# succinctlabs/sp1

Hardware: AMD Instinct MI355X
Metric: RISC-V cycles proved/sec (core shard prove): whole ShardProof of a full core shard of the reference's `fibonacci` guest, see config (higher is better)
Workload: dtype u32 (KoalaBear Montgomery words, exact integer arithmetic)

## Files before the change

sp1_amd/csrc/zc_compile.hpp:

```cpp
#pragma once
#include <memory>
#include <vector>

#include "common.hpp"
#include "zc_device.hpp"
#include "zc_poseidon2.hpp"
#include "zc_keccak.hpp"
#include "zc_mul.hpp"
#include "zc_poly.hpp"

namespace sp1hip {

using Ext = kb::Ext;
static inline Ext operator+(const Ext& a, const Ext& b) { return kb::ext_add(a, b); }
static inline Ext operator-(const Ext& a, const Ext& b) { return kb::ext_sub(a, b); }
static inline Ext operator*(const Ext& a, const Ext& b) { return kb::ext_mul(a, b); }

struct ZcMacro {
    uint32_t kind, base_col, first_constraint, aux0 = 0, aux1 = 0;
    uint32_t n_c = 0;
    uint32_t n_constraints() const { return kind == ZC_HINT_POLY ? n_c : kind == ZC_HINT_POSEIDON2 ? ZC_P2_CONSTRAINTS : kind == ZC_HINT_KECCAK ? ZC_KK_CONSTRAINTS : kind == ZC_HINT_MUL ? ZC_MUL_CONSTRAINTS : kind == ZC_HINT_SEPTIC_CURVE ? 7u : 14u; }
    uint32_t n_pieces() const { return kind == ZC_HINT_POLY ? 1u : kind == ZC_HINT_POSEIDON2 ? ZC_P2_PIECES : kind == ZC_HINT_KECCAK ? ZC_KK_PIECES : kind == ZC_HINT_MUL ? ZC_MUL_PIECES : kind == ZC_HINT_SEPTIC_CURVE ? 2u : 4u; }
    uint32_t n_host_pieces() const { return kind == ZC_HINT_SEPTIC_CURVE ? 1u : kind == ZC_HINT_SEPTIC_SUM ? 2u : n_pieces(); }
    void owned(uint32_t* lo, uint32_t* n) const {
        if (kind == ZC_HINT_POLY) { *lo = 0; *n = 0; }
        else if (kind == ZC_HINT_POSEIDON2) { *lo = base_col; *n = ZC_P2_COLUMNS; }
        else if (kind == ZC_HINT_KECCAK) { *lo = base_col; *n = ZC_KK_COLUMNS; }
        else if (kind == ZC_HINT_MUL) { *lo = base_col + MUL_CARRY; *n = ZC_MUL_OWNED; }
        else if (kind == ZC_HINT_SEPTIC_CURVE) { *lo = base_col; *n = 14; }
        else { *lo = aux0; *n = 28; }
    }
};

struct Chunk {
    std::vector<uint32_t> prog;
    uint32_t n_regs = 1, alpha_off = 0;
};

struct ZcPlan {
    uint32_t n_instr = 0, main_w = 0, prep_w = 0;
    bool macros_enabled = true;
    bool mul_enabled = true;
    std::vector<uint32_t> source;
    std::vector<uint32_t> prog;
    uint32_t n_regs = 1;
    std::vector<Chunk> chunks, mono, fine;
    std::vector<uint32_t> sched;
    std::vector<ZcMacro> macros;
    std::vector<ZcPoly> polys;
    std::vector<std::vector<ZcPolySeg>> poly_segs;
};

constexpr uint32_t ZC_FINE_LIMIT = 32, ZC_FINE_MAX_TERMS = 64;

int zc_get_plan(const uint32_t* program, uint32_t n_instr, uint32_t main_width, uint32_t prep_width, int chip_index,
                std::shared_ptr<const ZcPlan>* out, uint64_t rows = ~0ull);

Ext zc_eval_zero_row(const ZcPlan& plan, const Ext* alpha_pows, const uint32_t* publics);

}
```

sp1_amd/csrc/zc_kernels.hpp:

```cpp
#pragma once
#include "device_ctx.hpp"
#include "round_sync.hpp"
#include "zc_device.hpp"
#include "zc_poseidon2.hpp"
#include "zc_keccak.hpp"
#include "zc_mul.hpp"
#include "zc_poly.hpp"

namespace sp1hip {

template <bool FIRST, int MAXR> struct RegFile;

typedef uint32_t zc_lds_word_t __attribute__((address_space(3)));
typedef uint32_t zc_lds_quad_t __attribute__((ext_vector_type(4), address_space(3)));
typedef uint32_t zc_quad_t __attribute__((ext_vector_type(4)));
template <> struct RegFile<true, 0> {
    zc_lds_word_t* base;
    uint32_t stride;
    __device__ __forceinline__ uint32_t get(uint32_t i) const { return base[i * stride]; }
    __device__ __forceinline__ void set(uint32_t i, uint32_t v) { base[i * stride] = v; }
};
template <> struct RegFile<false, 0> {
    zc_lds_quad_t* base;
    uint32_t stride;
// ... 437 lines not shown
            const uint32_t k = threadIdx.x;
            partial[((size_t)bid * ZC_BIV_NODES + 4 * grp + n) * 8 + k] = kb::add(kb::add(red[k], red[8 + k]), kb::add(red[16 + k], red[24 + k]));
        }
    }
}

constexpr uint32_t ZC_CORNER_COLS = 32;
__global__ __launch_bounds__(256) void zc_biv_corner_kernel(const ZcDesc* __restrict__ descs, int n_descs, const uint32_t* __restrict__ eq,
                                                            uint32_t eq_len, uint32_t* __restrict__ partial, uint32_t block_base) {
    using K = KT<true>;
    __shared__ uint32_t red[4 * 16];
    const uint32_t bid = block_base + blockIdx.x;
    const ZcDesc d = zc_find_desc(descs, n_descs, bid);
    const uint32_t c0 = d.aux0, c1 = d.aux1;
    const uint32_t quads = (d.rows + 3) / 4;
    kb::Ext sb[4] = {kb::ext_zero(), kb::ext_zero(), kb::ext_zero(), kb::ext_zero()};
    for (uint32_t base = (bid - d.block_start) * d.block_pairs; base < quads; base += d.n_blocks * d.block_pairs)
    for (uint32_t i = base + threadIdx.x; i < min(base + d.block_pairs, quads); i += blockDim.x) {
        kb::Ext e;
#pragma unroll
        for (int k = 0; k < 4; k++) e.c[k] = eq[(size_t)k * eq_len + i];
        kb::Ext vb[4] = {kb::ext_zero(), kb::ext_zero(), kb::ext_zero(), kb::ext_zero()};
#pragma unroll 4
        for (uint32_t c = c0; c < c1; c++) {
            const kb::Ext pw = load_ext_aos(d.gkr_pows, c);
            const uint32_t* tbl = c < d.main_w ? d.main : d.prep;
            const uint32_t col = c < d.main_w ? c : c - d.main_w;
#pragma unroll
            for (uint32_t n = 0; n < 4; n++)
                if (4 * i + n < d.rows) vb[n] = kb::ext_add(vb[n], K::scale(pw, K::load(tbl, col, d.rows, 4 * i + n)));
        }
#pragma unroll
        for (int n = 0; n < 4; n++) sb[n] = kb::ext_add(sb[n], kb::ext_mul(vb[n], e));
    }
    const int lane = threadIdx.x & 63, wave = threadIdx.x >> 6;
#pragma unroll
    for (int n = 0; n < 4; n++)
#pragma unroll
        for (int k = 0; k < 4; k++) {
            const uint32_t w = zc_wave_sum(sb[n].c[k]);
            if (lane == 0) red[wave * 16 + 4 * n + k] = w;
        }
    __syncthreads();
    if (threadIdx.x < ZC_BIV_NODES * 8) {
        const uint32_t node = threadIdx.x / 8, k = threadIdx.x % 8;
        uint32_t v = 0;
        if (node < 4 && k >= 4) {
            const uint32_t j = 4 * node + (k - 4);
            v = kb::add(kb::add(red[j], red[16 + j]), kb::add(red[32 + j], red[48 + j]));
        }
        partial[((size_t)bid * ZC_BIV_NODES + node) * 8 + k] = v;
    }
}

template <uint32_t KIND>
__global__ __launch_bounds__(256) void zc_biv_macro_kernel(const ZcDesc* __restrict__ descs, int n_descs, const uint32_t* __restrict__ eq,
                                                           uint32_t eq_len, uint32_t* __restrict__ partial, uint32_t block_base,
                                                           const p2::RoundConstants* __restrict__ rc_p) {
    using K = KT<true>;
    __shared__ uint32_t red[32];
    if (threadIdx.x < 32) red[threadIdx.x] = 0;
    const uint32_t bid = block_base + blockIdx.x / (uint32_t)ZC_BIV_NODES;
    const uint32_t node = blockIdx.x % (uint32_t)ZC_BIV_NODES;
    const ZcBivNode nd = zc_biv_node(node);
    const ZcDesc d = zc_find_desc(descs, n_descs, bid);
    const uint32_t q = (d.flags >> 8) & 15u, base_col = d.pad;
    const auto* rc = (const p2::RoundConstants __attribute__((address_space(4)))*)(uintptr_t)rc_p;
    __syncthreads();
    const uint32_t quads = (d.rows + 3) / 4;
    kb::Ext sa = kb::ext_zero();
    for (uint32_t base = (bid - d.block_start) * d.block_pairs; base < quads; base += d.n_blocks * d.block_pairs)
    for (uint32_t i = base + threadIdx.x; i < min(base + d.block_pairs, quads); i += blockDim.x) {
        kb::Ext e;
#pragma unroll
        for (int k = 0; k < 4; k++) e.c[k] = eq[(size_t)k * eq_len + i];
        kb::Ext va = kb::ext_zero();
        auto ld_at = [&](uint32_t col, bool) -> uint32_t { return zc_biv_leaf(d.main, col, d.rows, i, nd); };
        auto ld = [&](uint32_t c, bool owned) -> uint32_t { return ld_at(base_col + c, owned); };
        auto sink = [&](uint32_t j, const uint32_t& v) { va = kb::ext_add(va, K::scale(load_ext_aos(d.alpha_pows, d.alpha_off + j), v)); };
        auto alpha = [&](uint32_t j) -> kb::Ext { return load_ext_aos(d.alpha_pows, d.alpha_off + j); };
        auto emit = [&](const kb::Ext& v) { va = kb::ext_add(va, v); };
        if constexpr (KIND == ZC_HINT_POSEIDON2) zc_p2_piece<P2Base>(q, rc, ld, sink);
        else if constexpr (KIND == ZC_HINT_KECCAK) zc_keccak_piece<P2Base>(q, ld, sink);
        else if constexpr (KIND == ZC_HINT_MUL) zc_mul_piece<P2Base>(q, ld, [&](uint32_t c, bool owned) -> uint32_t { return ld_at(d.aux0 + c, owned); }, sink);
        else if constexpr (KIND == ZC_HINT_SEPTIC_CURVE) zc_septic_curve_piece_w<P2Base, K>(q, ld, alpha, emit);
        else zc_septic_sum_piece_w<P2Base, K>(q, ld, [&](uint32_t c, bool owned) -> uint32_t { return ld_at(d.aux0 + c, owned); },
                                              [&]() -> uint32_t { return ld_at(d.aux1, false); }, alpha, emit);
        sa = kb::ext_add(sa, kb::ext_mul(va, e));
    }
    const int lane = threadIdx.x & 63, wave = threadIdx.x >> 6;
    uint32_t v[4];
#pragma unroll
    for (int k = 0; k < 4; k++) v[k] = zc_wave_sum(sa.c[k]);
    __syncthreads();
    if (lane == 0) {
#pragma unroll
        for (int k = 0; k < 4; k++) red[wave * 8 + k] = v[k];
    }
    __syncthreads();
    if (threadIdx.x < 8) {
        const uint32_t k = threadIdx.x;
        partial[((size_t)bid * ZC_BIV_NODES + node) * 8 + k] = k < 4 ? kb::add(kb::add(red[k], red[8 + k]), kb::add(red[16 + k], red[24 + k])) : 0u;
    }
}

struct ZcPolyTable {
    zc_const_words_t tb;
    __device__ __forceinline__ uint32_t word(uint32_t off) const { return tb[off]; }
    __device__ __forceinline__ kb::Ext coef(uint32_t off) const { return kb::Ext{{tb[off + 4], tb[off + 5], tb[off + 6], tb[off + 7]}}; }
};
__device__ __forceinline__ kb::Ext zc_ext_times_pow2(kb::Ext v, uint32_t k) {
    if (k == 0) return kb::ext_zero();
    for (uint32_t m = 1; m < k; m <<= 1) v = kb::ext_add(v, v);
    return v;
}
template <bool FIRST>
__global__ __launch_bounds__(256) void zc_poly_kernel(const ZcDesc* __restrict__ descs, int n_descs, const uint32_t* __restrict__ eq,
                                                      uint32_t eq_len, uint32_t* __restrict__ partial, uint32_t block_base) {
    using K = KT<FIRST>;
    using T = typename K::T;
    __shared__ uint32_t red[4 * 24];
    const uint32_t bid = block_base + blockIdx.x;
    const ZcDesc d = zc_find_desc(descs, n_descs, bid);
    const ZcPolyTable tab{(zc_const_words_t)(uintptr_t)d.prog};
    const uint32_t n_terms = tab.word(0), n_rest = tab.word(1), n_owned = tab.word(2);
    const uint32_t terms = (d.rows + 1) / 2;
    kb::Ext sa[3] = {kb::ext_zero(), kb::ext_zero(), kb::ext_zero()}, sb[2] = {kb::ext_zero(), kb::ext_zero()};
    for (uint32_t base = (bid - d.block_start) * d.block_pairs; base < terms; base += d.n_blocks * d.block_pairs)
    for (uint32_t i = base + threadIdx.x; i < min(base + d.block_pairs, terms); i += blockDim.x) {
        kb::Ext e;
#pragma unroll
        for (int k = 0; k < 4; k++) e.c[k] = eq[(size_t)k * eq_len + i];
        const bool has1 = 2 * i + 1 < d.rows;
        uint32_t off = ZC_POLY_HDR;
        auto form = [&](uint32_t n, kb::Ext& f0, kb::Ext& f1) {
            f0 = f1 = tab.coef(off);
            off += ZC_POLY_ENTRY;
#pragma unroll 4
            for (uint32_t k = 0; k < n; k++, off += ZC_POLY_ENTRY) {
                const uint32_t col = tab.word(off);
                const kb::Ext c = tab.coef(off);
                const T x0 = K::load(d.main, col, d.rows, 2 * i);
                const T x1 = has1 ? K::load(d.main, col, d.rows, 2 * i + 1) : K::zero();
                f0 = kb::ext_add(f0, K::scale(c, x0));
                f1 = kb::ext_add(f1, K::scale(c, x1));
            }
        };
        kb::Ext v0 = kb::ext_zero(), v2 = kb::ext_zero(), v4 = kb::ext_zero();
        for (uint32_t t = 0; t < n_terms; t++) {
            kb::Ext a0, a1, b0, b1;
            form(tab.word(4 + 3 * t), a0, a1);
            form(tab.word(5 + 3 * t), b0, b1);
            a0 = kb::ext_mul(a0, e); a1 = kb::ext_mul(a1, e);
            const kb::Ext da = kb::ext_sub(a1, a0), db = kb::ext_sub(b1, b0);
            const kb::Ext da2 = kb::ext_add(da, da), db2 = kb::ext_add(db, db);
            const kb::Ext a2 = kb::ext_add(a0, da2), b2 = kb::ext_add(b0, db2);
            kb::Ext p0 = FIRST ? kb::ext_zero() : kb::ext_mul(a0, b0), p2 = kb::ext_mul(a2, b2), p4 = kb::ext_mul(kb::ext_add(a2, da2), kb::ext_add(b2, db2));
            const uint32_t n2 = tab.word(6 + 3 * t);
            if (n2 != ZC_POLY_NONE) {
                kb::Ext c0, c1;
                form(n2, c0, c1);
                const kb::Ext dc = kb::ext_sub(c1, c0), dc2 = kb::ext_add(dc, dc), c2 = kb::ext_add(c0, dc2);
                if (!FIRST) p0 = kb::ext_mul(p0, c0);
                p2 = kb::ext_mul(p2, c2);
                p4 = kb::ext_mul(p4, kb::ext_add(c2, dc2));
            }
            v0 = kb::ext_add(v0, p0); v2 = kb::ext_add(v2, p2); v4 = kb::ext_add(v4, p4);
// ... 209 lines not shown
        for (int k = 0; k < 4; k++) rr[k] = kb::ext_mul(rr[k], e);
        slopes(rr);
#pragma unroll
        for (int n = 0; n < ZC_BIV_NODES; n++) sa[n] = kb::ext_add(sa[n], at(rr, zc_biv_node(n)));
    }
    const int lane = threadIdx.x & 63, wave = threadIdx.x >> 6;
    uint32_t v[48];
#pragma unroll
    for (int n = 0; n < ZC_BIV_NODES; n++)
#pragma unroll
        for (int k = 0; k < 4; k++) v[n * 4 + k] = zc_wave_sum(sa[n].c[k]);
    if (lane == 0) {
#pragma unroll
        for (int k = 0; k < 48; k++) red[wave * 48 + k] = v[k];
    }
    __syncthreads();
    if (threadIdx.x < 48) {
        const uint32_t k = threadIdx.x;
        uint32_t acc = red[k];
        for (uint32_t w = 1; w < blockDim.x / 64; w++) acc = kb::add(acc, red[w * 48 + k]);
        partial[((size_t)bid * ZC_BIV_NODES + k / 4) * 8 + (k & 3u)] = acc;
        partial[((size_t)bid * ZC_BIV_NODES + k / 4) * 8 + 4 + (k & 3u)] = 0u;
    }
}

struct P2Base4 {
    using T = kb::Ext;
    static __device__ __forceinline__ T add(const T& a, const T& b) { return kb::ext_add(a, b); }
    static __device__ __forceinline__ T sub(const T& a, const T& b) { return kb::ext_sub(a, b); }
    static __device__ __forceinline__ T mul(const T& a, const T& b) { return KT4::mul(a, b); }
    static __device__ __forceinline__ T addc(const T& a, uint32_t c) { return KC4::addc(a, c); }
    static __device__ __forceinline__ T mulc(const T& a, uint32_t c) { return kb::ext_mul_base(a, c); }
};
__global__ __launch_bounds__(256) void zc_biv_keccak_kernel(const ZcDesc* __restrict__ descs, int n_descs, const uint32_t* __restrict__ eq,
                                                            uint32_t eq_len, uint32_t* __restrict__ partial, uint32_t block_base) {
    using K = KT<true>;
    __shared__ uint32_t red[4][32];
    const uint32_t bid = block_base + blockIdx.x / ZC_BIV_GROUPS;
    const uint32_t grp = blockIdx.x % ZC_BIV_GROUPS;
    const ZcBivNode n0 = zc_biv_node(4 * grp), n1 = zc_biv_node(4 * grp + 1), n2 = zc_biv_node(4 * grp + 2), n3 = zc_biv_node(4 * grp + 3);
    const ZcDesc d = zc_find_desc(descs, n_descs, bid);
    const uint32_t q = (d.flags >> 8) & 15u, base_col = d.pad;
    const uint32_t quads = (d.rows + 3) / 4;
    kb::Ext sa[4] = {kb::ext_zero(), kb::ext_zero(), kb::ext_zero(), kb::ext_zero()};
    for (uint32_t base = (bid - d.block_start) * d.block_pairs; base < quads; base += d.n_blocks * d.block_pairs)
    for (uint32_t i = base + threadIdx.x; i < min(base + d.block_pairs, quads); i += blockDim.x) {
        kb::Ext e;
#pragma unroll
        for (int k = 0; k < 4; k++) e.c[k] = eq[(size_t)k * eq_len + i];
        kb::Ext va[4] = {kb::ext_zero(), kb::ext_zero(), kb::ext_zero(), kb::ext_zero()};
        auto ld = [&](uint32_t c, bool) -> kb::Ext {
            const zc_global_words_t g = (zc_global_words_t)d.main + (size_t)(base_col + c) * d.rows;
            const uint32_t r = 4 * i;
            const uint32_t r00 = g[r], r01 = r + 1 < d.rows ? g[r + 1] : 0u, r10 = r + 2 < d.rows ? g[r + 2] : 0u, r11 = r + 3 < d.rows ? g[r + 3] : 0u;
            return kb::Ext{{zc_biv_interp(r00, r01, r10, r11, n0), zc_biv_interp(r00, r01, r10, r11, n1), zc_biv_interp(r00, r01, r10, r11, n2),
                            zc_biv_interp(r00, r01, r10, r11, n3)}};
        };
        auto sink = [&](uint32_t j, const kb::Ext& v) {
            const kb::Ext a = load_ext_aos(d.alpha_pows, d.alpha_off + j);
#pragma unroll
            for (int n = 0; n < 4; n++) va[n] = kb::ext_add(va[n], K::scale(a, v.c[n]));
        };
        zc_keccak_piece<P2Base4>(q, ld, sink);
#pragma unroll
        for (int n = 0; n < 4; n++) sa[n] = kb::ext_add(sa[n], kb::ext_mul(va[n], e));
    }
    const int lane = threadIdx.x & 63, wave = threadIdx.x >> 6;
#pragma unroll
    for (int n = 0; n < 4; n++)
#pragma unroll
        for (int k = 0; k < 4; k++) {
            const uint32_t v = zc_wave_sum(sa[n].c[k]);
            if (lane == 0) red[wave][n * 4 + k] = v;
        }
    __syncthreads();
    if (threadIdx.x < 32) {
        const uint32_t n = threadIdx.x >> 3, k = threadIdx.x & 7u;
        const uint32_t w = n * 4 + (k & 3u);
        partial[((size_t)bid * ZC_BIV_NODES + 4 * grp + n) * 8 + k] =
            k < 4 ? kb::add(kb::add(red[0][w], red[1][w]), kb::add(red[2][w], red[3][w])) : 0u;
    }
}

constexpr uint32_t ZC_BIV_SUM_WORDS = 68;
__global__ __launch_bounds__(256) void zc_biv_reduce_kernel(const ZcChipRange* __restrict__ ranges, const uint32_t* __restrict__ partial,
                                                            const uint32_t* __restrict__ eq, uint32_t eq_len,
                                                            uint32_t* __restrict__ out, RoundSync rs, uint32_t seq) {
    __shared__ uint32_t acc[32][8];
    const uint32_t range = blockIdx.x / (uint32_t)ZC_BIV_NODES, node = blockIdx.x % (uint32_t)ZC_BIV_NODES;
    const ZcChipRange d = ranges[range];
    const uint32_t word = threadIdx.x & 7u, grp = threadIdx.x >> 3;
    {
        const uint32_t* p = partial + ((size_t)d.block_start * ZC_BIV_NODES + node) * 8 + word;
        uint32_t a[4] = {0, 0, 0, 0};
        uint32_t b = grp;
        for (; b + 96 < d.n_blocks; b += 128)
#pragma unroll
            for (int u = 0; u < 4; u++) a[u] = kb::add(a[u], p[(size_t)(b + 32 * u) * (ZC_BIV_NODES * 8)]);
        for (; b < d.n_blocks; b += 32) a[0] = kb::add(a[0], p[(size_t)b * (ZC_BIV_NODES * 8)]);
        acc[grp][word] = kb::add(kb::add(a[0], a[1]), kb::add(a[2], a[3]));
    }
    __syncthreads();
    if (threadIdx.x < 12) {
        const uint32_t w = threadIdx.x;
        uint32_t val = 0, dst = 0xffffffffu;
        if (w < 8) {
            for (uint32_t g = 0; g < 32; g++) val = kb::add(val, acc[g][w]);
            if (w < 4) dst = 4 * node + w;
            else if (node < 4) dst = 48 + 4 * node + (w - 4);
        } else if (node == 0) {
            const uint32_t k = w - 8;
            val = d.th < eq_len ? eq[(size_t)k * eq_len + d.th] : 0u;
            dst = 64 + k;
        }
        if (dst != 0xffffffffu) {
            out[(size_t)range * ZC_BIV_SUM_WORDS + dst] = val;
            if (rs.host_slot != nullptr)
                __hip_atomic_store(const_cast<uint32_t*>(rs.host_slot) + 1 + (size_t)range * ZC_BIV_SUM_WORDS + dst, val, __ATOMIC_RELAXED, __HIP_MEMORY_SCOPE_SYSTEM);
        }
    }
    if (rs.host_slot == nullptr) return;
    asm volatile("s_waitcnt vmcnt(0)" ::: "memory");
    __syncthreads();
    if (threadIdx.x == 0 && rs_ticket_is_last_acq_rel(rs.counter, blockIdx.x, gridDim.x)) rs_publish_seq(rs.host_slot, seq);
}

template <bool FIRST>
__global__ __launch_bounds__(256) void zc_reduce_kernel(const ZcChipRange* __restrict__ ranges, const uint32_t* __restrict__ partial,
                                                        const uint32_t* __restrict__ eq, uint32_t eq_len,
                                                        uint32_t* __restrict__ out, RoundSync rs, uint32_t seq) {
    __shared__ uint32_t acc[10][24];
    const ZcChipRange d = ranges[blockIdx.x];
    uint32_t y0, y2, y4, e;
    zc_reduce_range<FIRST>(d, partial, eq, eq_len, acc, y0, y2, y4, e);
    if (threadIdx.x < 4) {
        const uint32_t k = threadIdx.x;
        uint32_t* o = out + (size_t)blockIdx.x * 16;
        o[k] = y0; o[4 + k] = y2; o[8 + k] = y4;
        o[12 + k] = e;
    }
    if (rs.host_slot != nullptr) zc_store_host_sums(rs.host_slot, blockIdx.x, y0, y2, y4, e);
    if (rs.host_slot == nullptr) return;
    asm volatile("s_waitcnt vmcnt(0)" ::: "memory");
    __syncthreads();
    if (threadIdx.x == 0 && rs_ticket_is_last_acq_rel(rs.counter, blockIdx.x, gridDim.x)) rs_publish_seq(rs.host_slot, seq);
}

constexpr uint32_t ZC_FIX_ROWS = 2048;
template <bool FIRST>
__global__ __launch_bounds__(256) void zc_fix_kernel(const ZcFixDesc* __restrict__ descs, int n_descs, kb::Ext alpha) {
    using K = KT<FIRST>;
    int lo = 0, hi = n_descs - 1;
    while (lo < hi) {
        const int mid = (lo + hi + 1) >> 1;
        if (__builtin_amdgcn_readfirstlane(descs[mid].block_start) <= blockIdx.x) lo = mid; else hi = mid - 1;
    }
    const ZcFixDesc d = descs[lo];
    const uint32_t out_rows = (d.rows + 1) / 2;
    const uint32_t lb = blockIdx.x - d.block_start;
    uint32_t c = d.bpc == 1 ? lb : __umulhi(lb, d.bpc_magic);
    uint32_t tile = lb - c * d.bpc;
    if (tile >= d.bpc) { tile -= d.bpc; c++; }
    if (tile >= d.bpc) { tile -= d.bpc; c++; }
    const uint32_t i0 = tile * ZC_FIX_ROWS, i1 = min(out_rows, i0 + ZC_FIX_ROWS);
    for (uint32_t i = i0 + threadIdx.x; i < i1; i += 256u) {
        typename K::T x = K::load(d.in, c, d.rows, 2 * i);
// ... 44 lines not shown
```

sp1_amd/csrc/zc_mul.hpp:

```cpp
#pragma once
#include "zc_poseidon2.hpp"

namespace sp1hip {

constexpr uint32_t ZC_HINT_MUL = 6;
constexpr uint32_t ZC_MUL_CONSTRAINTS = 16, ZC_MUL_PIECES = 2, ZC_MUL_OWNED = 16;
constexpr uint32_t MUL_CARRY = 0, MUL_PRODUCT = 16, MUL_B_LOW = 32, MUL_C_LOW = 36, MUL_B_SE = 43, MUL_C_SE = 44, MUL_FLAGS = 45, MUL_COLUMNS = 50;
constexpr uint32_t MUL_OPC_FROM_OPB = 7;
constexpr uint32_t MUL_INV256 = 0x7e810001u;

template <class F, class LD, class LDX, class SINK>
KB_HD void zc_mul_piece(uint32_t q, LD&& ld, LDX&& ldx, SINK&& sink) {
    using T = typename F::T;
    const uint32_t inv256 = kb::to_monty(MUL_INV256), c255 = kb::to_monty(255u), c256 = kb::to_monty(256u);
    T xb[8], yb[8];
#pragma unroll
    for (uint32_t i = 0; i < 4; i++) {
        const T xl = ld(MUL_B_LOW + i, false), yl = ld(MUL_C_LOW + i, false);
        xb[2 * i] = xl; xb[2 * i + 1] = F::mulc(F::sub(ldx(i, false), xl), inv256);
        yb[2 * i] = yl; yb[2 * i + 1] = F::mulc(F::sub(ldx(MUL_OPC_FROM_OPB + i, false), yl), inv256);
    }
    const T se_b = F::mulc(ld(MUL_B_SE, false), c255), se_c = F::mulc(ld(MUL_C_SE, false), c255);
    T is_real = ld(MUL_FLAGS, false);
#pragma unroll
    for (uint32_t i = 1; i < 5; i++) is_real = F::add(is_real, ld(MUL_FLAGS + i, false));
    T px = xb[0], py = yb[0];
#pragma unroll
    for (uint32_t k = 0; k < 16; k++) {
        if (k > 8) { px = F::add(px, xb[k - 8]); py = F::add(py, yb[k - 8]); }
        if ((k & 1u) != q) continue;
        const uint32_t i0 = k > 7 ? k - 7 : 0, i1 = k < 7 ? k : 7;
        T m = k >= 8 ? F::add(F::mul(se_c, px), F::mul(se_b, py)) : F::mul(xb[0], yb[k]);
#pragma unroll
        for (uint32_t i = (k >= 8 ? i0 : 1u); i <= i1; i++) m = F::add(m, F::mul(xb[i], yb[k - i]));
        T v = F::add(F::sub(ld(MUL_PRODUCT + k, false), m), F::mulc(ld(MUL_CARRY + k, true), c256));
        if (k > 0) v = F::sub(v, ld(MUL_CARRY + k - 1, false));
        sink(k, F::mul(is_real, v));
    }
}

}
```

sp1_amd/csrc/zerocheck.hip:

```cpp
#include <algorithm>
#include <array>
#include <chrono>
#include <cstring>
#include <memory>
#include <vector>

#include "zc_compile.hpp"
#include "zc_kernels.hpp"

namespace sp1hip {

constexpr uint32_t ZC_MONO_MIN_TERMS = 1024;
constexpr uint32_t ZC_FORK_MAX_BLOCKS = 1u << 30;
constexpr uint32_t ZC_MAX_PAIRS = 131072;
constexpr uint32_t ZC_SMALL_ROUND_WGS = 16384;
constexpr int ZC_FORK_STREAMS = 3, ZC_N_FORK = 2;

static Ext ext_c(uint32_t canonical) { return kb::ext_from_base(kb::to_monty(canonical)); }
using UniPoly = std::vector<Ext>;

struct VGeq {
    uint32_t threshold;
    Ext geq_c, eq_c;
    VGeq fix(const Ext& alpha) const {
// ... 552 lines not shown
            size_t chunk_words = 0, mono_words = 0;
            for (auto& ck : c.chunks) chunk_words += ck.prog.size();
            for (auto& ck : c.mono) mono_words += ck.prog.size();
            use_mono[i] = c.chunks.size() > 1 && terms >= ZC_MONO_MIN_TERMS && mono_wg != 0 && 2 * chunk_words > 3 * mono_words;
            if (!use_mono[i] && terms <= ZC_FINE_MAX_TERMS && c.fine.size() > c.chunks.size()) use_mono[i] = 2;
            const std::vector<Chunk>& cks = use_mono[i] == 1 ? c.mono : use_mono[i] == 2 ? c.fine : c.chunks;
            uint32_t regs = 1, instr = 1;
            for (auto& ck : cks) { regs = std::max(regs, ck.n_regs); instr = std::max<uint32_t>(instr, (uint32_t)(ck.prog.size() / 4)); }
            const uint32_t stage_max = (uint32_t)env_uint("SP1HIP_ZC_STAGE_MAX", 0);
            bool staged = instr <= stage_max;
            uint32_t wg = (r == 0 && !biv) ? zc_wg_for<true>(regs, staged ? 128 + (size_t)instr * 16 : 128) : zc_wg_for<false>(regs, staged ? 128 + (size_t)instr * 16 : 128);
            if (wg == 0 && use_mono[i] != 2) {
                use_mono[i] = 2;
                regs = 1; instr = 1;
                for (auto& ck : c.fine) { regs = std::max(regs, ck.n_regs); instr = std::max<uint32_t>(instr, (uint32_t)(ck.prog.size() / 4)); }
                staged = instr <= stage_max;
                wg = (r == 0 && !biv) ? zc_wg_for<true>(regs, staged ? 128 + (size_t)instr * 16 : 128) : zc_wg_for<false>(regs, staged ? 128 + (size_t)instr * 16 : 128);
            }
            SP1HIP_REQUIRE(wg != 0, "constraint program too large: one constraint keeps more than 160 extension values live (the LDS register file of one wave)");
            uint32_t resident = 0;
            if (terms > ZC_FINE_MAX_TERMS) {
                const size_t per_wg = (staged ? 128 + (size_t)instr * 16 : 128) + ((r == 0 && !biv) ? zc_rf_lane_bytes<true>(regs) : zc_rf_lane_bytes<false>(regs)) * wg;
                resident = (uint32_t)std::min<size_t>(ZC_LDS_CU / per_wg, 2048 / wg);
            }
            size_t g = 0;
            for (; g < groups.size(); g++) if (groups[g].staged == staged && groups[g].wg == wg && groups[g].resident == resident) break;
            if (g == groups.size()) groups.push_back(Group{staged, wg, resident, 1, 1, 0, 0, {}});
            groups[g].max_regs = std::max(groups[g].max_regs, regs);
            groups[g].max_instr = std::max(groups[g].max_instr, instr);
            groups[g].chips.push_back(i);
        }
        uint32_t& total_blocks = rp.total_blocks;
        total_blocks = 0;
        for (auto& g : groups) {
            g.block_lo = total_blocks;
            for (int i : g.chips) {
                ChipState& c = *st[i];
                const uint32_t terms = (uint32_t)((vrows[i] + unit - 1) / unit);
                const uint32_t bp = g.wg ? g.wg : 256u;
                uint32_t blocks = (terms + bp - 1) / bp;
                if (blocks > ZC_MAX_PAIRS / bp) blocks = std::max(1u, ZC_MAX_PAIRS / bp);
                const std::vector<Chunk>& cks = use_mono[i] == 1 ? c.mono : use_mono[i] == 2 ? c.fine : c.chunks;
                const std::vector<uint32_t>& offs = use_mono[i] == 1 ? c.mono_off : use_mono[i] == 2 ? c.fine_off : c.chunk_off;
                ZcChipRange rg{total_blocks, 0, biv ? (uint32_t)(vrows[i] / 4) : terms - 1, 0};
                for (size_t q = 0; q < cks.size(); q++) {
                    ZcDesc d{};
                    d.prog = c.p_prog + (size_t)offs[q] * 4;
                    d.n_instr = (uint32_t)(cks[q].prog.size() / 4);
                    d.main = vmain[i]; d.prep = vprep[i]; d.main_w = c.in->main_width; d.prep_w = c.in->prep_width;
                    d.rows = (uint32_t)vrows[i]; d.alpha_pows = c.p_alpha; d.gkr_pows = c.p_gkr;
                    d.block_start = total_blocks; d.n_blocks = blocks;
                    d.alpha_off = cks[q].alpha_off; d.flags = (q == 0 && !biv) ? 1u : 0u;
                    d.block_pairs = bp;
                    total_blocks += blocks;
                    descs.push_back(d);
                }
                rg.n_blocks = total_blocks - rg.block_start;
                ranges.push_back(rg);
                desc_chip.push_back(i);
            }
            g.n_blocks = total_blocks - g.block_lo;
        }
        uint32_t (&macro_lo)[ZC_MACRO_KINDS + 1] = rp.macro_lo;
        uint32_t (&macro_n)[ZC_MACRO_KINDS + 1] = rp.macro_n;
        {
            uint64_t max_terms = 0;
            for (int i = 0; i < n_chips; i++)
                for (const ZcMacro& m : st[i]->macros) if (m.kind == ZC_HINT_POLY && vrows[i]) max_terms = std::max<uint64_t>(max_terms, (vrows[i] + unit - 1) / unit);
            rp.poly_wave = !biv && r > 0 && max_terms > 0 && max_terms <= ZC_POLY_WAVE_MAX_TERMS;
        }
        for (uint32_t kind = ZC_HINT_POSEIDON2; kind < ZC_MACRO_KINDS; kind++) {
            if (kind == ZC_MACRO_BOTH_SEPTIC) continue;
            macro_lo[kind] = total_blocks;
            for (int i = 0; i < n_chips; i++) {
                ChipState& c = *st[i];
                if (vrows[i] == 0) continue;
                const uint32_t terms = (uint32_t)((vrows[i] + unit - 1) / unit);
                const bool wave_form = kind == ZC_HINT_POLY && rp.poly_wave;
                const uint32_t blocks = wave_form ? std::min<uint32_t>((terms + 3) / 4, 1024u) : std::min<uint32_t>((terms + 255) / 256, 512u);
                ZcChipRange rg{total_blocks, 0, biv ? (uint32_t)(vrows[i] / 4) : terms - 1, 0};
                for (size_t mi = 0; mi < c.macros.size(); mi++) {
                    const ZcMacro& m = c.macros[mi];
                    if (m.kind != kind) continue;
                    for (uint32_t q = 0; q < m.n_pieces(); q++) {
                        ZcDesc d{};
                        if (kind == ZC_HINT_POLY) d.prog = c.p_blob + c.poly_off[mi];
                        d.main = vmain[i]; d.prep = vprep[i]; d.main_w = c.in->main_width; d.prep_w = c.in->prep_width;
                        d.rows = (uint32_t)vrows[i]; d.alpha_pows = c.p_alpha; d.gkr_pows = c.p_gkr;
                        d.block_start = total_blocks; d.n_blocks = blocks;
                        d.alpha_off = m.first_constraint; d.flags = ZC_DESC_MACRO | (q << 8) | (m.kind << 12);
                        d.block_pairs = wave_form ? 4 : 256; d.pad = m.base_col; d.aux0 = m.aux0; d.aux1 = m.aux1;
                            total_blocks += blocks;
                        descs.push_back(d);
                    }
                }
                rg.n_blocks = total_blocks - rg.block_start;
                if (rg.n_blocks) { ranges.push_back(rg); desc_chip.push_back(i); }
            }
            macro_n[kind] = total_blocks - macro_lo[kind];
        }
        macro_lo[ZC_RANGE_CORNERS] = total_blocks;
        if (biv)
            for (int i = 0; i < n_chips; i++) {
                ChipState& c = *st[i];
                if (vrows[i] == 0) continue;
                const uint32_t quads = (uint32_t)((vrows[i] + 3) / 4), width = c.in->main_width + c.in->prep_width;
                const uint32_t blocks = std::min<uint32_t>((quads + 255) / 256, 512u);
                ZcChipRange rg{total_blocks, 0, (uint32_t)(vrows[i] / 4), 0};
                for (uint32_t c0 = 0; c0 < width; c0 += ZC_CORNER_COLS) {
                    ZcDesc d{};
                    d.main = vmain[i]; d.prep = vprep[i]; d.main_w = c.in->main_width; d.prep_w = c.in->prep_width;
                    d.rows = (uint32_t)vrows[i]; d.alpha_pows = c.p_alpha; d.gkr_pows = c.p_gkr;
                    d.block_start = total_blocks; d.n_blocks = blocks;
                    d.flags = ZC_DESC_MACRO | (ZC_RANGE_CORNERS << 12);
                    d.block_pairs = 256; d.aux0 = c0; d.aux1 = std::min(width, c0 + ZC_CORNER_COLS);
                    total_blocks += blocks;
                    descs.push_back(d);
                }
                rg.n_blocks = total_blocks - rg.block_start;
                if (rg.n_blocks) { ranges.push_back(rg); desc_chip.push_back(i); }
            }
        macro_n[ZC_RANGE_CORNERS] = total_blocks - macro_lo[ZC_RANGE_CORNERS];
        std::vector<ZcFixDesc>& fds = rp.fds;
        std::vector<uint32_t*>& fresh = rp.fresh;
        std::vector<std::pair<int, bool>>& owner = rp.owner;
        uint32_t& fix_blocks = rp.fix_blocks;
        fix_blocks = 0;
        size_t fold_words = 0;
        uint32_t* const fold_base = (uint32_t*)d_fold[biv ? 1 : (r & 1)].p;
        for (int i = 0; i < n_chips; i++) {
            ChipState& c = *st[i];
            if (vrows[i] == 0) continue;
            const uint64_t out_rows = (vrows[i] + unit - 1) / unit;
            for (int which = 0; which < 2; which++) {
                const uint32_t width = which == 0 ? c.in->main_width : c.in->prep_width;
                if (width == 0) continue;
                uint32_t* const nb = fold_base + fold_words;
                fold_words += ((size_t)out_rows * width * 4 + 3) & ~(size_t)3;
                ZcFixDesc fd{};
                fd.in = which == 0 ? vmain[i] : vprep[i];
                fd.out = nb;
                fd.rows = (uint32_t)vrows[i]; fd.width = width; fd.block_start = fix_blocks;
                fd.bpc = (uint32_t)((out_rows + ZC_FIX_ROWS - 1) / ZC_FIX_ROWS);
                fd.bpc_magic = (uint32_t)((((uint64_t)1 << 32) / fd.bpc) & 0xffffffffull);
                fd.n_blocks = fd.bpc * width;
                fix_blocks += fd.n_blocks;
                fds.push_back(fd);
                fresh.push_back(nb);
                owner.push_back({i, which == 0});
            }
        }
        const size_t off_ranges = rp.off_ranges = (descs.size() * sizeof(ZcDesc) + 15) & ~(size_t)15;
        const size_t off_fds = rp.off_fds = (off_ranges + ranges.size() * sizeof(ZcChipRange) + 15) & ~(size_t)15;
        const size_t pack_bytes = rp.pack_bytes = off_fds + fds.size() * sizeof(ZcFixDesc);
        std::vector<uint8_t>& pack = rp.pack;
        pack.assign(std::max<size_t>(pack_bytes, 16), 0);
        if (!descs.empty()) memcpy(pack.data(), descs.data(), descs.size() * sizeof(ZcDesc));
        if (!ranges.empty()) memcpy(pack.data() + off_ranges, ranges.data(), ranges.size() * sizeof(ZcChipRange));
        if (!fds.empty()) memcpy(pack.data() + off_fds, fds.data(), fds.size() * sizeof(ZcFixDesc));
        rp.rows_next = vrows; rp.main_next = vmain; rp.prep_next = vprep;
        for (size_t k = 0; k < fds.size(); k++) {
            if (owner[k].second) rp.main_next[owner[k].first] = fresh[k]; else rp.prep_next[owner[k].first] = fresh[k];
        }
        for (int i = 0; i < n_chips; i++) if (rp.rows_next[i]) rp.rows_next[i] = (rp.rows_next[i] + unit - 1) / unit;
        return SP1HIP_SUCCESS;
    }
    int upload_plan(const RoundPlan& rp, int which) {
// ... 4 lines not shown
        }
        return stage.upload(d_descs2[which].p, rp.pack.data(), rp.pack_bytes);
    }
    int plan_next(int r) {
        if (r >= L || (int)plans.size() > r) return SP1HIP_SUCCESS;
        if (r == 0) {
            std::vector<uint64_t> rows0(n_chips);
            std::vector<const uint32_t*> main0(n_chips), prep0(n_chips);
            for (int i = 0; i < n_chips; i++) { rows0[i] = tr.chip[i].rows; main0[i] = st[i]->d_main; prep0[i] = st[i]->d_prep; }
            plans.emplace_back(new RoundPlan());
            SP1HIP_TRY(plan_round(0, rows0, main0, prep0, *plans.back(), bivariate));
            return upload_plan(*plans.back(), bivariate ? 1 : 0);
        }
        const RoundPlan& prev = *plans.back();
        while ((int)plans.size() <= r) plans.emplace_back(new RoundPlan());
        SP1HIP_TRY(plan_round(r, prev.rows_next, prev.main_next, prev.prep_next, *plans.back(), false));
        return upload_plan(*plans.back(), r & 1);
    }
    PlanViews device_plan(const RoundPlan& rp, int which) const {
        const uint8_t* base = (const uint8_t*)d_descs2[which].p;
        return PlanViews{(const ZcDesc*)base, (const ZcChipRange*)(base + rp.off_ranges), (const ZcFixDesc*)(base + rp.off_fds)};
    }

    template <class LaunchReduce>
    int publish_and_wait(size_t n_words, const void* d_src, uint32_t* h_out, int next_round, LaunchReduce&& launch_reduce) {
        const bool direct = n_words + 1 <= MAILBOX_WORDS;
        const RoundSync rs_pub = direct ? RoundSync{rsync.d_counter, (volatile uint32_t*)mb.h_slot} : RoundSync{};
        if (direct) { rsync.pending = true; mb.pending = true; }
        SP1HIP_TRY(launch_reduce(rs_pub));
        SP1HIP_TRY(plan_next(next_round));
        timer.lap(ZcTimer::PLAN);
        if (direct) { SP1HIP_TRY(mb.wait_next(h_out, n_words)); rsync.pending = false; }
        else SP1HIP_TRY(mb.fetch(d_src, n_words, h_out));
        timer.lap(ZcTimer::WAIT);
        return SP1HIP_SUCCESS;
    }
    void apply_fix(const RoundPlan& rp) {
        for (size_t k = 0; k < rp.fds.size(); k++) {
            ChipState& c = *st[rp.owner[k].first];
            if (rp.owner[k].second) c.d_main = rp.fresh[k]; else c.d_prep = rp.fresh[k];
        }
    }

    int bivariate_sums(const RoundPlan& rp, std::vector<uint32_t>& bsums) {
        const uint32_t eq_len = 1u << (L - 2);
        const uint32_t* d_eq = d_eq_all.u32() + 4 * (((size_t)1 << (L - 2)) - 1);
        const int n_descs = (int)rp.descs.size(), n_ranges = (int)rp.ranges.size();
        const PlanViews dp = device_plan(rp, 1);
        const ZcDesc* dd = dp.descs;
        partial_cap = (size_t)rp.total_blocks * ZC_BIV_NODES * 8 * 4;
        SP1HIP_TRY(d_partial.alloc(partial_cap, s));
        DevBuf d_bsums;
        SP1HIP_TRY(d_bsums.alloc(bsums.size() * 4, s));
        ScopedTimer tm("zerocheck_round", s);
        RoundFork fork;
        SP1HIP_TRY(fork.begin(s, fork_enabled && rp.n_launches() > 1 && active_provers() <= 1));
        hipStream_t ls;
        {
            std::vector<size_t> by_work(rp.groups.size());
            for (size_t g = 0; g < by_work.size(); g++) by_work[g] = g;
            auto work = [&](size_t g) { return (double)rp.groups[g].n_blocks * (double)rp.groups[g].max_instr; };
            std::stable_sort(by_work.begin(), by_work.end(), [&](size_t a, size_t b) { return work(a) > work(b); });
            double load0 = 0, load2 = 0;
            for (size_t gi : by_work) {
                const auto& g = rp.groups[gi];
                const int slot = load0 <= load2 ? 0 : 2;
                (slot == 0 ? load0 : load2) += work(gi);
                SP1HIP_TRY(fork.stream_of(slot, &ls));
                SP1HIP_TRY(launch_biv_round(g, dd, n_descs, d_eq, eq_len, d_publics.u32(), d_partial.u32(), ls));
            }
        }
#define SP1HIP_ZC_BIV_MACRO_LAUNCH(KIND, SLOT)                                                                                           \
        if (rp.macro_n[KIND]) {                                                                                                \
            SP1HIP_TRY(fork.stream_of(SLOT, &ls));                                                                             \
            hipLaunchKernelGGL((zc_biv_macro_kernel<KIND>), dim3(rp.macro_n[KIND] * (uint32_t)ZC_BIV_NODES), dim3(256), 0, ls, dd, n_descs, d_eq, eq_len, d_partial.u32(), rp.macro_lo[KIND], ctx->d_rc); \
            SP1HIP_LAUNCH_CHECK();                                                                                             \
        }
        if (rp.macro_n[ZC_HINT_KECCAK]) {
            SP1HIP_TRY(fork.stream_of(1, &ls));
            hipLaunchKernelGGL(zc_biv_keccak_kernel, dim3(rp.macro_n[ZC_HINT_KECCAK] * ZC_BIV_GROUPS), dim3(256), 0, ls, dd, n_descs, d_eq, eq_len, d_partial.u32(), rp.macro_lo[ZC_HINT_KECCAK]);
            SP1HIP_LAUNCH_CHECK();
        }
        SP1HIP_ZC_BIV_MACRO_LAUNCH(3u, 2)
        SP1HIP_ZC_BIV_MACRO_LAUNCH(6u, 1)
        SP1HIP_ZC_BIV_MACRO_LAUNCH(1u, 1)
        if (rp.macro_n[ZC_HINT_POLY]) {
            SP1HIP_TRY(fork.stream_of(1, &ls));
            hipLaunchKernelGGL(zc_biv_poly_kernel, dim3(rp.macro_n[ZC_HINT_POLY]), dim3(256), 0, ls, dd, n_descs, d_eq, eq_len, d_partial.u32(), rp.macro_lo[ZC_HINT_POLY]);
            SP1HIP_LAUNCH_CHECK();
        }
        if (rp.macro_n[ZC_RANGE_CORNERS]) {
            SP1HIP_TRY(fork.stream_of(1, &ls));
            hipLaunchKernelGGL(zc_biv_corner_kernel, dim3(rp.macro_n[ZC_RANGE_CORNERS]), dim3(256), 0, ls, dd, n_descs, d_eq, eq_len, d_partial.u32(), rp.macro_lo[ZC_RANGE_CORNERS]);
            SP1HIP_LAUNCH_CHECK();
        }
        SP1HIP_ZC_BIV_MACRO_LAUNCH(2u, 1)
#undef SP1HIP_ZC_BIV_MACRO_LAUNCH
        SP1HIP_TRY(fork.join());
        return publish_and_wait((size_t)n_ranges * ZC_BIV_SUM_WORDS, d_bsums.p, bsums.data(), 2, [&](const RoundSync& rs_pub) -> int {
            hipLaunchKernelGGL(zc_biv_reduce_kernel, dim3(n_ranges * ZC_BIV_NODES), dim3(256), 0, s, dp.ranges, d_partial.u32(), d_eq, eq_len, d_bsums.u32(), rs_pub, mb.seq + 1);
            SP1HIP_LAUNCH_CHECK();
            return SP1HIP_SUCCESS;
        });
    }
    int run_bivariate_rounds() {
        const RoundPlan& rp = *plans[0];
        std::vector<uint32_t> bsums((size_t)std::max<size_t>(rp.ranges.size(), 1) * ZC_BIV_SUM_WORDS);
        if (!rp.descs.empty()) SP1HIP_TRY(bivariate_sums(rp, bsums));
        SP1HIP_TRY(plan_next(2));
        std::vector<BivNodes> H(n_chips);
        assemble_biv_nodes(rp.desc_chip, bsums, tr.chip, H);
        const CubicBasis& cubic = cubic_basis();
        std::vector<std::array<Ext, 3>> hv(n_chips);
        const Ext zX = zeta[L - 2], zY = zeta[L - 1];
        for (int i = 0; i < n_chips; i++) {
            if (tr.chip[i].rows == 0) continue;
            for (int k = 0; k < 3; k++) { const int t = k == 0 ? 0 : k + 1; hv[i][k] = (kb::ext_one() - zX) * H[i][0][t] + zX * H[i][1][t]; }
        }
        const Ext a0 = tr.round_messages(zY, hv);
        tr.update_claims();
        Ext Lk[4];
        for (int k = 0; k < 4; k++) {
            Ext acc = kb::ext_from_base(cubic.c[k][3]);
            for (int d = 2; d >= 0; d--) acc = acc * a0 + kb::ext_from_base(cubic.c[k][d]);
            Lk[k] = acc;
        }
        for (int i = 0; i < n_chips; i++) {
            const ChipClaim& c = tr.chip[i];
            if (c.rows == 0) continue;
            for (int k = 0; k < 3; k++) {
                const int t = k == 0 ? 0 : k + 1;
                const Ext v = H[i][t][0] * Lk[0] + H[i][t][1] * Lk[1] + H[i][t][2] * Lk[2] + H[i][t][3] * Lk[3];
                hv[i][k] = c.eq_adj * v;
            }
        }
        const Ext a1 = tr.round_messages(zX, hv);
        timer.lap(ZcTimer::UNI);
        if (!rp.fds.empty()) {
            ScopedTimer tm("zerocheck_fix", s);
            hipLaunchKernelGGL(zc_fix2_kernel, dim3(rp.fix_blocks), dim3(256), 0, s, device_plan(rp, 1).fds, (int)rp.fds.size(), a0, a1);
            SP1HIP_LAUNCH_CHECK();
            apply_fix(rp);
        }
        tr.update_claims();
        tr.fold_rows(4);
        return SP1HIP_SUCCESS;
    }

    struct Launch { int kind; size_t group; double est; int slot; };
    static void order_launches(const RoundPlan& rp, int r, bool forked, std::vector<Launch>& order) {
        const std::vector<Group>& groups = rp.groups;
        const uint32_t* macro_n = rp.macro_n;
        static const double floor_us[ZC_MACRO_KINDS] = {45.0, 75.0, 45.0, 60.0, 60.0, 120.0, 45.0, 90.0};
        for (size_t g = 0; g < groups.size(); g++) order.push_back({0, g, floor_us[0] * (1.0 + groups[g].n_blocks * 3 / 1024.0 * std::max(groups[g].max_instr, 25u) / 100.0), 0});
        const bool both_septic = forked && r > 0 && macro_n[2] && macro_n[3] && (uint64_t)rp.total_blocks * 3 <= ZC_SMALL_ROUND_WGS;
        for (int kind = 1; kind <= 3; kind++) {
            if (!macro_n[kind] || (both_septic && kind == 2)) continue;
            if (both_septic && kind == 3) order.push_back({(int)ZC_MACRO_BOTH_SEPTIC, 0, floor_us[3] * (1.0 + (macro_n[2] + macro_n[3]) * 3 / 1024.0), 0});
            else order.push_back({kind, 0, floor_us[kind] * (1.0 + macro_n[kind] * 3 / 1024.0), 0});
        }
        if (macro_n[ZC_HINT_KECCAK]) order.push_back({(int)ZC_HINT_KECCAK, 0, floor_us[ZC_HINT_KECCAK] * (1.0 + macro_n[ZC_HINT_KECCAK] * 3 / 1024.0), 0});
        if (macro_n[ZC_HINT_MUL]) order.push_back({(int)ZC_HINT_MUL, 0, floor_us[ZC_HINT_MUL] * (1.0 + macro_n[ZC_HINT_MUL] * 3 / 1024.0), 0});
        if (macro_n[ZC_HINT_POLY]) order.push_back({(int)ZC_HINT_POLY, 0, floor_us[ZC_HINT_POLY] * (1.0 + macro_n[ZC_HINT_POLY] * 3 / 1024.0), 0});
        if (forked) {
            std::stable_sort(order.begin(), order.end(), [](const Launch& a, const Launch& b) { return a.est > b.est; });
            double load[ZC_FORK_STREAMS + 1] = {0, 7, 14, 21};
            for (Launch& ln : order) {
// ... 226 lines not shown
```

Baseline: 97.36 million.

## Add dedicated bivariate MUL zerocheck kernel evaluating all nodes per thread

Replaces the generic per-node bivariate macro kernel for MUL chips, which ran one block per node and piece, with a dedicated kernel. Each thread loads the four rows of a quad once, precomputes the bilinear operand coefficients, and loops over all 12 nodes while accumulating into LDS. Both constraint pieces are also merged into one. This cuts the repeated global loads and operand reconstruction done for every node, at the cost of heavy LDS use (12x256 quads) and higher register pressure, which the waves_per_eu hint tries to keep in check.

```diff
diff --git a/sp1_amd/csrc/zc_compile.hpp b/sp1_amd/csrc/zc_compile.hpp
--- a/sp1_amd/csrc/zc_compile.hpp
+++ b/sp1_amd/csrc/zc_compile.hpp
@@ -20,7 +20,7 @@
     uint32_t kind, base_col, first_constraint, aux0 = 0, aux1 = 0;
     uint32_t n_c = 0;
     uint32_t n_constraints() const { return kind == ZC_HINT_POLY ? n_c : kind == ZC_HINT_POSEIDON2 ? ZC_P2_CONSTRAINTS : kind == ZC_HINT_KECCAK ? ZC_KK_CONSTRAINTS : kind == ZC_HINT_MUL ? ZC_MUL_CONSTRAINTS : kind == ZC_HINT_SEPTIC_CURVE ? 7u : 14u; }
-    uint32_t n_pieces() const { return kind == ZC_HINT_POLY ? 1u : kind == ZC_HINT_POSEIDON2 ? ZC_P2_PIECES : kind == ZC_HINT_KECCAK ? ZC_KK_PIECES : kind == ZC_HINT_MUL ? ZC_MUL_PIECES : kind == ZC_HINT_SEPTIC_CURVE ? 2u : 4u; }
+    uint32_t n_pieces(bool biv = false) const { return kind == ZC_HINT_POLY ? 1u : kind == ZC_HINT_POSEIDON2 ? ZC_P2_PIECES : kind == ZC_HINT_KECCAK ? ZC_KK_PIECES : kind == ZC_HINT_MUL ? (biv ? 1u : ZC_MUL_PIECES) : kind == ZC_HINT_SEPTIC_CURVE ? 2u : 4u; }
     uint32_t n_host_pieces() const { return kind == ZC_HINT_SEPTIC_CURVE ? 1u : kind == ZC_HINT_SEPTIC_SUM ? 2u : n_pieces(); }
     void owned(uint32_t* lo, uint32_t* n) const {
         if (kind == ZC_HINT_POLY) { *lo = 0; *n = 0; }
diff --git a/sp1_amd/csrc/zc_kernels.hpp b/sp1_amd/csrc/zc_kernels.hpp
--- a/sp1_amd/csrc/zc_kernels.hpp
+++ b/sp1_amd/csrc/zc_kernels.hpp
@@ -543,7 +543,6 @@
         auto emit = [&](const kb::Ext& v) { va = kb::ext_add(va, v); };
         if constexpr (KIND == ZC_HINT_POSEIDON2) zc_p2_piece<P2Base>(q, rc, ld, sink);
         else if constexpr (KIND == ZC_HINT_KECCAK) zc_keccak_piece<P2Base>(q, ld, sink);
-        else if constexpr (KIND == ZC_HINT_MUL) zc_mul_piece<P2Base>(q, ld, [&](uint32_t c, bool owned) -> uint32_t { return ld_at(d.aux0 + c, owned); }, sink);
         else if constexpr (KIND == ZC_HINT_SEPTIC_CURVE) zc_septic_curve_piece_w<P2Base, K>(q, ld, alpha, emit);
         else zc_septic_sum_piece_w<P2Base, K>(q, ld, [&](uint32_t c, bool owned) -> uint32_t { return ld_at(d.aux0 + c, owned); },
                                               [&]() -> uint32_t { return ld_at(d.aux1, false); }, alpha, emit);
@@ -919,6 +918,94 @@
     }
 }
 
+typedef const zc_quad_t __attribute__((address_space(1)))* zc_global_quads_t;
+typedef const char __attribute__((address_space(1)))* zc_global_bytes_t;
+template <bool ALIGNED>
+__device__ __forceinline__ kb::Ext zc_biv_rows(const uint32_t* tbl, uint32_t col, uint32_t rows, uint32_t q) {
+    const zc_global_bytes_t g = (zc_global_bytes_t)((zc_global_words_t)tbl + (size_t)col * rows);
+    if constexpr (ALIGNED) {
+        const zc_quad_t v = *(zc_global_quads_t)(g + 16u * q);
+        return kb::Ext{{v.x, v.y, v.z, v.w}};
+    } else {
+        const uint32_t r = 4 * q, last = rows - 1;
+        const uint32_t x0 = *(zc_global_words_t)(g + 4u * r), x1 = *(zc_global_words_t)(g + 4u * min(r + 1, last));
+        const uint32_t x2 = *(zc_global_words_t)(g + 4u * min(r + 2, last)), x3 = *(zc_global_words_t)(g + 4u * min(r + 3, last));
+        return kb::Ext{{x0, r + 1 <= last ? x1 : 0u, r + 2 <= last ? x2 : 0u, r + 3 <= last ? x3 : 0u}};
+    }
+}
+template <bool ALIGNED>
+__device__ __forceinline__ void zc_biv_mul_quad(const ZcDesc& d, uint32_t i, const kb::Ext& e, zc_lds_quad_t* my_sums) {
+    using K = KT<true>;
+    const uint32_t base_col = d.pad;
+    ZcMulOperands<P2Base4> f;
+    zc_mul_operands<P2Base4>([&](uint32_t c, bool) -> kb::Ext { return zc_biv_rows<ALIGNED>(d.main, base_col + c, d.rows, i); },
+                             [&](uint32_t c, bool) -> kb::Ext { return zc_biv_rows<ALIGNED>(d.main, d.aux0 + c, d.rows, i); }, f);
+#pragma unroll
+    for (uint32_t w = 0; w < ZC_MUL_OPERANDS; w++) {
+        const uint32_t dy = kb::sub(f.w[w].c[1], f.w[w].c[0]), dx = kb::sub(f.w[w].c[2], f.w[w].c[0]);
+        f.w[w].c[3] = kb::sub(kb::sub(f.w[w].c[3], f.w[w].c[2]), dy);
+        f.w[w].c[1] = dy; f.w[w].c[2] = dx;
+    }
+#pragma unroll 1
+    for (uint32_t n = 0; n < (uint32_t)ZC_BIV_NODES; n++) {
+        const ZcBivNode nd = zc_biv_node(n);
+        ZcMulOperands<P2Base> o;
+#pragma unroll
+        for (uint32_t w = 0; w < ZC_MUL_OPERANDS; w++)
+            o.w[w] = zc_reduce36((uint64_t)f.w[w].c[0] + (uint64_t)nd.cx * f.w[w].c[2] + (uint64_t)nd.cy * f.w[w].c[1] + (uint64_t)nd.cxy * f.w[w].c[3]);
+        kb::Ext va = kb::ext_zero();
+        uint32_t iq = i;
+        asm volatile("" : "+v"(iq));
+        zc_mul_constraints<P2Base>(ZC_MUL_ALL, o, [&](uint32_t c, bool) -> uint32_t {
+                                       const kb::Ext r = zc_biv_rows<ALIGNED>(d.main, base_col + c, d.rows, iq);
+                                       return zc_biv_interp(r.c[0], r.c[1], r.c[2], r.c[3], nd);
+                                   },
+                                   [&](uint32_t j, const uint32_t& v) {
+                                       va = kb::ext_add(va, K::scale(load_ext_aos(d.alpha_pows, d.alpha_off + j), v));
+                                       if (j & 1u) { asm volatile("" ::: "memory"); __builtin_amdgcn_sched_barrier(0); }
+                                   });
+        const zc_quad_t s = my_sums[n * 256];
+        const kb::Ext t = kb::ext_add(kb::Ext{{s.x, s.y, s.z, s.w}}, kb::ext_mul(va, e));
+        my_sums[n * 256] = zc_quad_t{t.c[0], t.c[1], t.c[2], t.c[3]};
+    }
+}
+__global__ __launch_bounds__(256) __attribute__((amdgpu_waves_per_eu(2))) void zc_biv_mul_kernel(const ZcDesc* __restrict__ descs, int n_descs, const uint32_t* __restrict__ eq,
+                                                         uint32_t eq_len, uint32_t* __restrict__ partial, uint32_t block_base) {
+    __shared__ zc_quad_t sums[ZC_BIV_NODES][256];
+    __shared__ uint32_t red[4][ZC_BIV_NODES * 4];
+    zc_lds_quad_t* const my_sums = (zc_lds_quad_t*)&sums[0][0] + threadIdx.x;
+    const uint32_t bid = block_base + blockIdx.x;
+    const ZcDesc d = zc_find_desc(descs, n_descs, bid);
+    const uint32_t quads = (d.rows + 3) / 4;
+    const bool aligned = (d.rows & 3u) == 0 && ((uintptr_t)d.main & 15u) == 0;
+#pragma unroll
+    for (int n = 0; n < ZC_BIV_NODES; n++) my_sums[n * 256] = zc_quad_t{0u, 0u, 0u, 0u};
+    for (uint32_t base = (bid - d.block_start) * d.block_pairs; base < quads; base += d.n_blocks * d.block_pairs)
+    for (uint32_t i = base + threadIdx.x; i < min(base + d.block_pairs, quads); i += blockDim.x) {
+        kb::Ext e;
+#pragma unroll
+        for (int k = 0; k < 4; k++) e.c[k] = eq[(size_t)k * eq_len + i];
+        if (aligned) zc_biv_mul_quad<true>(d, i, e, my_sums);
+        else zc_biv_mul_quad<false>(d, i, e, my_sums);
+    }
+    const int lane = threadIdx.x & 63, wave = threadIdx.x >> 6;
+#pragma unroll
+    for (int n = 0; n < ZC_BIV_NODES; n++) {
+        const zc_quad_t s = my_sums[n * 256];
+        const uint32_t v[4] = {zc_wave_sum(s.x), zc_wave_sum(s.y), zc_wave_sum(s.z), zc_wave_sum(s.w)};
+        if (lane == 0) {
+#pragma unroll
+            for (int k = 0; k < 4; k++) red[wave][n * 4 + k] = v[k];
+        }
+    }
+    __syncthreads();
+    if (threadIdx.x < ZC_BIV_NODES * 8) {
+        const uint32_t n = threadIdx.x >> 3, k = threadIdx.x & 7u;
+        const uint32_t w = n * 4 + (k & 3u);
+        partial[((size_t)bid * ZC_BIV_NODES + n) * 8 + k] = k < 4 ? kb::add(kb::add(red[0][w], red[1][w]), kb::add(red[2][w], red[3][w])) : 0u;
+    }
+}
+
 constexpr uint32_t ZC_BIV_SUM_WORDS = 68;
 __global__ __launch_bounds__(256) void zc_biv_reduce_kernel(const ZcChipRange* __restrict__ ranges, const uint32_t* __restrict__ partial,
                                                             const uint32_t* __restrict__ eq, uint32_t eq_len,
diff --git a/sp1_amd/csrc/zc_mul.hpp b/sp1_amd/csrc/zc_mul.hpp
--- a/sp1_amd/csrc/zc_mul.hpp
+++ b/sp1_amd/csrc/zc_mul.hpp
@@ -5,38 +5,58 @@
 
 constexpr uint32_t ZC_HINT_MUL = 6;
 constexpr uint32_t ZC_MUL_CONSTRAINTS = 16, ZC_MUL_PIECES = 2, ZC_MUL_OWNED = 16;
+constexpr uint32_t ZC_MUL_ALL = 2;
 constexpr uint32_t MUL_CARRY = 0, MUL_PRODUCT = 16, MUL_B_LOW = 32, MUL_C_LOW = 36, MUL_B_SE = 43, MUL_C_SE = 44, MUL_FLAGS = 45, MUL_COLUMNS = 50;
 constexpr uint32_t MUL_OPC_FROM_OPB = 7;
 constexpr uint32_t MUL_INV256 = 0x7e810001u;
 
-template <class F, class LD, class LDX, class SINK>
-KB_HD void zc_mul_piece(uint32_t q, LD&& ld, LDX&& ldx, SINK&& sink) {
+constexpr uint32_t MULO_B = 0, MULO_C = 8, MULO_SE_B = 16, MULO_SE_C = 17, MULO_IS_REAL = 18, ZC_MUL_OPERANDS = 19;
+template <class F> struct ZcMulOperands { typename F::T w[ZC_MUL_OPERANDS]; };
+
+template <class F, class LD, class LDX>
+KB_HD void zc_mul_operands(LD&& ld, LDX&& ldx, ZcMulOperands<F>& o) {
     using T = typename F::T;
-    const uint32_t inv256 = kb::to_monty(MUL_INV256), c255 = kb::to_monty(255u), c256 = kb::to_monty(256u);
-    T xb[8], yb[8];
+    const uint32_t inv256 = kb::to_monty(MUL_INV256), c255 = kb::to_monty(255u);
 #pragma unroll
     for (uint32_t i = 0; i < 4; i++) {
         const T xl = ld(MUL_B_LOW + i, false), yl = ld(MUL_C_LOW + i, false);
-        xb[2 * i] = xl; xb[2 * i + 1] = F::mulc(F::sub(ldx(i, false), xl), inv256);
-        yb[2 * i] = yl; yb[2 * i + 1] = F::mulc(F::sub(ldx(MUL_OPC_FROM_OPB + i, false), yl), inv256);
+        o.w[MULO_B + 2 * i] = xl; o.w[MULO_B + 2 * i + 1] = F::mulc(F::sub(ldx(i, false), xl), inv256);
+        o.w[MULO_C + 2 * i] = yl; o.w[MULO_C + 2 * i + 1] = F::mulc(F::sub(ldx(MUL_OPC_FROM_OPB + i, false), yl), inv256);
     }
-    const T se_b = F::mulc(ld(MUL_B_SE, false), c255), se_c = F::mulc(ld(MUL_C_SE, false), c255);
+    o.w[MULO_SE_B] = F::mulc(ld(MUL_B_SE, false), c255);
+    o.w[MULO_SE_C] = F::mulc(ld(MUL_C_SE, false), c255);
     T is_real = ld(MUL_FLAGS, false);
 #pragma unroll
     for (uint32_t i = 1; i < 5; i++) is_real = F::add(is_real, ld(MUL_FLAGS + i, false));
+    o.w[MULO_IS_REAL] = is_real;
+}
+
+template <class F, class LD, class SINK>
+KB_HD void zc_mul_constraints(uint32_t q, const ZcMulOperands<F>& o, LD&& ld, SINK&& sink) {
+    using T = typename F::T;
+    const uint32_t c256 = kb::to_monty(256u);
+    const T* xb = o.w + MULO_B;
+    const T* yb = o.w + MULO_C;
     T px = xb[0], py = yb[0];
 #pragma unroll
     for (uint32_t k = 0; k < 16; k++) {
         if (k > 8) { px = F::add(px, xb[k - 8]); py = F::add(py, yb[k - 8]); }
-        if ((k & 1u) != q) continue;
+        if (q != ZC_MUL_ALL && (k & 1u) != q) continue;
         const uint32_t i0 = k > 7 ? k - 7 : 0, i1 = k < 7 ? k : 7;
-        T m = k >= 8 ? F::add(F::mul(se_c, px), F::mul(se_b, py)) : F::mul(xb[0], yb[k]);
+        T m = k >= 8 ? F::add(F::mul(o.w[MULO_SE_C], px), F::mul(o.w[MULO_SE_B], py)) : F::mul(xb[0], yb[k]);
 #pragma unroll
         for (uint32_t i = (k >= 8 ? i0 : 1u); i <= i1; i++) m = F::add(m, F::mul(xb[i], yb[k - i]));
         T v = F::add(F::sub(ld(MUL_PRODUCT + k, false), m), F::mulc(ld(MUL_CARRY + k, true), c256));
         if (k > 0) v = F::sub(v, ld(MUL_CARRY + k - 1, false));
-        sink(k, F::mul(is_real, v));
+        sink(k, F::mul(o.w[MULO_IS_REAL], v));
     }
 }
 
+template <class F, class LD, class LDX, class SINK>
+KB_HD void zc_mul_piece(uint32_t q, LD&& ld, LDX&& ldx, SINK&& sink) {
+    ZcMulOperands<F> o;
+    zc_mul_operands<F>(ld, ldx, o);
+    zc_mul_constraints<F>(q, o, ld, sink);
 }
+
+}
diff --git a/sp1_amd/csrc/zerocheck.hip b/sp1_amd/csrc/zerocheck.hip
--- a/sp1_amd/csrc/zerocheck.hip
+++ b/sp1_amd/csrc/zerocheck.hip
@@ -658,7 +658,7 @@
                 for (size_t mi = 0; mi < c.macros.size(); mi++) {
                     const ZcMacro& m = c.macros[mi];
                     if (m.kind != kind) continue;
-                    for (uint32_t q = 0; q < m.n_pieces(); q++) {
+                    for (uint32_t q = 0; q < m.n_pieces(biv); q++) {
                         ZcDesc d{};
                         if (kind == ZC_HINT_POLY) d.prog = c.p_blob + c.poly_off[mi];
                         d.main = vmain[i]; d.prep = vprep[i]; d.main_w = c.in->main_width; d.prep_w = c.in->prep_width;
@@ -829,7 +829,11 @@
             SP1HIP_LAUNCH_CHECK();
         }
         SP1HIP_ZC_BIV_MACRO_LAUNCH(3u, 2)
-        SP1HIP_ZC_BIV_MACRO_LAUNCH(6u, 1)
+        if (rp.macro_n[ZC_HINT_MUL]) {
+            SP1HIP_TRY(fork.stream_of(1, &ls));
+            hipLaunchKernelGGL(zc_biv_mul_kernel, dim3(rp.macro_n[ZC_HINT_MUL]), dim3(256), 0, ls, dd, n_descs, d_eq, eq_len, d_partial.u32(), rp.macro_lo[ZC_HINT_MUL]);
+            SP1HIP_LAUNCH_CHECK();
+        }
         SP1HIP_ZC_BIV_MACRO_LAUNCH(1u, 1)
         if (rp.macro_n[ZC_HINT_POLY]) {
             SP1HIP_TRY(fork.stream_of(1, &ls));
```

New measurement: 95.32 million. 0.979x the previous value.
